# automl/CARL

Measured on AMD Instinct MI355X. Metric: env-steps/sec (whole node) at 65k parallel contexts, 1/2/4/8 MI355X, higher is better.
Workload: dtype f32

## Files before the change

carl_amd/_lib.py:

```python
from __future__ import annotations

import ctypes as C
import os

import torch

from carl_amd import build as _build

CARL_ABI_VERSION = 9
CARL_MAX_CTX_OBS = 32

CARTPOLE, PENDULUM, ACROBOT, MOUNTAINCAR, MOUNTAINCAR_CONT = range(5)
CARL_N_FAMILIES = 5
ERR_INVALID_ARGUMENT, ERR_UNSUPPORTED = -1, -2
SEL_STATIC, SEL_ROUND_ROBIN, SEL_RANDOM, SEL_HOST = range(4)
FLAG_AUTORESET = 1
FLAG_CARTPOLE_RECOMPUTE = 2
FLAG_ACROBOT_FP32 = 4
FLAG_AUTORESET_FIRST_STATE = 8
FLAG_ROLLOUT_DIRECT = 16
FLAG_BRAX_GENERIC = 32
FLAG_BRAX_FP32 = 64
ROLLOUT_STAGED, ROLLOUT_DIRECT_SHAPE, ROLLOUT_DIRECT_FLAG = range(3)
ACTION_I32, ACTION_I64, ACTION_F32, ACTION_U8, ACTION_F16, ACTION_BF16 = range(6)

_vp = C.c_void_p


class FamilyInfo(C.Structure):
    _fields_ = [
        ("state_dim", C.c_int32), ("obs_dim", C.c_int32), ("n_features", C.c_int32),
        ("action_dim", C.c_int32), ("action_is_discrete", C.c_int32), ("n_actions", C.c_int32),
        ("max_episode_steps", C.c_int32), ("reserved", C.c_int32),
        ("action_low", C.c_float), ("action_high", C.c_float),
    ]


class Batch(C.Structure):
    _fields_ = [
        ("family", C.c_int32), ("n_lanes", C.c_int32), ("n_contexts", C.c_int32),
        ("ctx_stride", C.c_int32), ("max_episode_steps", C.c_int32), ("selector", C.c_int32),
        ("selector_stride", C.c_int32), ("flags", C.c_int32),
        ("lane_offset", C.c_int64), ("seed", C.c_uint64),
        ("state", _vp), ("elapsed", _vp), ("ctx_idx", _vp), ("episode", _vp), ("n_calls", _vp),
        ("ep_return", _vp),
        ("ctx_table", _vp), ("ctx_obs", _vp),
        ("n_ctx_obs", C.c_int32), ("ctx_obs_feat", C.c_int32 * CARL_MAX_CTX_OBS),
        ("fin_capacity", C.c_int32),
        ("last_return", _vp), ("last_length", _vp), ("episodes_done", _vp),
        ("fin_count", _vp), ("fin_lane", _vp), ("fin_return", _vp), ("fin_length", _vp),
        ("goal_pos", _vp), ("success", _vp), ("first_state", _vp),
    ]


class StepIO(C.Structure):
# ... 169 lines not shown
```

carl_amd/csrc/carl_amd.hip:

```cpp
#include <hip/hip_runtime.h>

#include <cstdarg>
#include <cstdio>
#include <cstdlib>
#include <cstring>
#include <map>
#include <mutex>
#include <utility>

#include "../../include/carl_amd.h"
#include "classic_control.hip.h"
#include "context_kernels.hip.h"
#include "engine_kernels.hip.h"
#include "host_common.hpp"

namespace carl_host {

thread_local char g_err[512] = "";

int fail(int code, const char* fmt, ...) {
  va_list ap;
  va_start(ap, fmt);
  vsnprintf(g_err, sizeof g_err, fmt, ap);
  va_end(ap);
// ... 64 lines not shown
  if (io == nullptr) return fail(CARL_ERR_INVALID_ARGUMENT, "%s: io is NULL", who);
  if (!io->action || !io->obs || !io->reward || !io->terminated || !io->truncated)
    return fail(CARL_ERR_INVALID_ARGUMENT, "%s: a required io pointer is NULL", who);
  const bool discrete = kInfo[b->family].action_is_discrete != 0;
  if (discrete && io->action_dtype != CARL_ACTION_I32 && io->action_dtype != CARL_ACTION_I64 &&
      io->action_dtype != CARL_ACTION_U8)
    return fail(CARL_ERR_INVALID_ARGUMENT, "%s: discrete family needs int32/int64 (carl_rollout: or uint8) actions", who);
  if (io->action_dtype == CARL_ACTION_U8 && (reinterpret_cast<uintptr_t>(io->action) & 3) != 0)
    return fail(CARL_ERR_INVALID_ARGUMENT, "%s: uint8 actions must be 4-byte aligned", who);
  const bool half = io->action_dtype == CARL_ACTION_F16 || io->action_dtype == CARL_ACTION_BF16;
  if (!discrete && io->action_dtype != CARL_ACTION_F32 && !half)
    return fail(CARL_ERR_INVALID_ARGUMENT, "%s: continuous family needs float32 (carl_rollout: or float16 / bfloat16) actions", who);
  if (half && (reinterpret_cast<uintptr_t>(io->action) & 7) != 0)
    return fail(CARL_ERR_INVALID_ARGUMENT, "%s: float16 / bfloat16 actions must be 8-byte aligned", who);
  if (io->row_pitch != 0 && io->row_pitch < b->n_lanes)
    return fail(CARL_ERR_INVALID_ARGUMENT, "%s: io.row_pitch %d < n_lanes %d (0 = dense rows)", who, io->row_pitch, b->n_lanes);
  return 0;
}

template <class Fam>
bool use_lds_ctx(const carl_batch_t* b) {
  const size_t bytes = (size_t)Fam::F * b->n_contexts * sizeof(float);
  return bytes <= 32 * 1024 && (int64_t)b->n_contexts * 8 <= (int64_t)b->n_lanes;
}

int row_pitch_of(const carl_batch_t* b, const carl_step_io_t* io) { return io->row_pitch > 0 ? io->row_pitch : b->n_lanes; }

struct RolloutPlan {
  int variant = CARL_ROLLOUT_STAGED;
  bool lean = false;
  bool unsupported = false;
  int ak = 0;
  bool plain = false, ldsctx = false, moves = false, fin = false, ar = false, deep = false;
  size_t lds_bytes = 0;
};

template <class Fam>
RolloutPlan plan_rollout(const carl_batch_t* b, const carl_step_io_t* io) {
  static_assert(carl::predraw_of<Fam>::value, "the staged kernels below are instantiated for predrawing families");
  RolloutPlan p;
  const int dt = io->action_dtype;
  p.ak = dt == CARL_ACTION_I64 ? 1 : dt == CARL_ACTION_U8 ? carl::kActU8 : dt == CARL_ACTION_F16 ? carl::kActF16
         : dt == CARL_ACTION_BF16 ? carl::kActBF16 : 0;
  const int pitch = row_pitch_of(b, io), n16 = (b->n_lanes + 15) / 16 * 16;
  const uintptr_t bits = reinterpret_cast<uintptr_t>(io->obs) | reinterpret_cast<uintptr_t>(io->reward) |
                         reinterpret_cast<uintptr_t>(io->terminated) | reinterpret_cast<uintptr_t>(io->truncated) |
                         reinterpret_cast<uintptr_t>(io->final_obs);
  const uintptr_t amask = p.ak == carl::kActU8 ? 3u : p.ak > carl::kActU8 ? 7u : 15u;
  const bool aligned = (bits & 15) == 0 && (reinterpret_cast<uintptr_t>(io->action) & amask) == 0;
  if (b->flags & CARL_FLAG_ROLLOUT_DIRECT)
    p.variant = CARL_ROLLOUT_DIRECT_FLAG;
  else if (!(aligned && pitch % 16 == 0 && (b->n_lanes % 16 == 0 || pitch == n16)))
    p.variant = CARL_ROLLOUT_DIRECT_SHAPE;
  const bool keeps_context = b->selector == CARL_SEL_STATIC || b->selector == CARL_SEL_HOST;
  p.lean = p.variant == CARL_ROLLOUT_STAGED && keeps_context && b->fin_count == nullptr && io->final_obs == nullptr;
  p.unsupported = p.ak >= carl::kActU8 && !p.lean;
  if (p.variant != CARL_ROLLOUT_STAGED) return p;

  p.lds_bytes = carl::rollout_staged_lds_bytes<Fam>();
  const size_t table_bytes = (size_t)Fam::F * b->n_contexts * sizeof(float);
  constexpr size_t static_lds = carl::has_tables<Fam>::value ? sizeof(double) * 2 * CARL_SINCOS_TAB_N : 0;
  const bool table_fits = use_lds_ctx<Fam>(b) && p.lds_bytes + table_bytes + static_lds <= 160 * 1024;
  if (p.lean) {
    p.plain = true;
    p.ar = carl::dense_done_of<Fam>::value && (b->flags & CARL_FLAG_AUTORESET);
    p.deep = p.ak == 0 && b->n_lanes < carl::deep_below_lanes_of<Fam>::value;
  } else if (carl::dense_done_of<Fam>::value && b->fin_count == nullptr) {
    p.plain = true;
    p.moves = !keeps_context;
    p.fin = io->final_obs != nullptr;
    p.ldsctx = p.moves && table_fits;
  } else {
    p.ldsctx = !keeps_context && table_fits;
  }
  if (p.ldsctx) p.lds_bytes += table_bytes;
  return p;
}

using staged_kern_t = void (*)(carl_batch_t, carl_step_io_t, int);

template <class Fam>
staged_kern_t staged_kernel(const RolloutPlan& p) {
#define CARL_STAGED(AK, PLAIN, LDSCTX, MOVES, FIN, AR, DEEP)                                                         \
  if (p.ak == AK && p.plain == PLAIN && p.ldsctx == LDSCTX && p.moves == MOVES && p.fin == FIN && p.ar == AR &&    \
      p.deep == DEEP)                                                                                              \
    return carl::rollout_staged_kernel<Fam, AK, bool(PLAIN), bool(LDSCTX), bool(MOVES), bool(FIN), bool(AR), bool(DEEP)>;
#define CARL_STAGED_01(...) CARL_STAGED(0, __VA_ARGS__) CARL_STAGED(1, __VA_ARGS__)
  constexpr bool dense = carl::dense_done_of<Fam>::value, deep = carl::deep_below_lanes_of<Fam>::value > 0;
  CARL_STAGED_01(    0,     0,    0,  0, 0,   0)
  CARL_STAGED_01(    0,     1,    0,  0, 0,   0)
  CARL_STAGED_01(    1,     0,    0,  0, 0,   0)
  if constexpr (std::is_same_v<typename Fam::Action, int>) {
    CARL_STAGED(carl::kActU8, 1, 0, 0, 0, 0, 0)
  } else {
    CARL_STAGED(carl::kActF16, 1, 0, 0, 0, 0, 0)
    CARL_STAGED(carl::kActBF16, 1, 0, 0, 0, 0, 0)
  }
  if constexpr (deep) CARL_STAGED(0, 1, 0, 0, 0, 0, 1)
  if constexpr (dense) {
    CARL_STAGED_01(  1,     0,    0,  0, 1,   0)
    CARL_STAGED(carl::kActU8, 1, 0, 0, 0, 1, 0)
    if constexpr (deep) CARL_STAGED(0, 1, 0, 0, 0, 1, 1)
    CARL_STAGED_01(  1,     0,    0,  1, 0,   0)
    CARL_STAGED_01(  1,     0,    1,  0, 0,   0)
    CARL_STAGED_01(  1,     0,    1,  1, 0,   0)
    CARL_STAGED_01(  1,     1,    1,  0, 0,   0)
    CARL_STAGED_01(  1,     1,    1,  1, 0,   0)
  }
#undef CARL_STAGED_01
#undef CARL_STAGED
  return nullptr;
}

int pick_block(int n, bool lds) { return (lds || n > 256 * 1024) ? 256 : 64; }

template <class Fam>
int launch_reset(const carl_batch_t* b, const uint8_t* mask, const int32_t* idx, const int32_t* count, float* obs,
                 hipStream_t s) {
  if (b->n_lanes == 0) return 0;
  const bool lds = use_lds_ctx<Fam>(b);
  const int block = 256;
  int grid = (b->n_lanes + block - 1) / block;
  if (grid > 4096) grid = 4096;
  if (lds) {
    const size_t sh = (size_t)Fam::F * b->n_contexts * sizeof(float);
    hipLaunchKernelGGL((carl::reset_kernel<Fam, true>), dim3(grid), dim3(block), sh, s, *b, mask, idx, count, obs);
  } else {
    hipLaunchKernelGGL((carl::reset_kernel<Fam, false>), dim3(grid), dim3(block), 0, s, *b, mask, idx, count, obs);
  }
  return check_launch("carl_reset");
}

template <class Fam>
int launch_step(const carl_batch_t* b, const carl_step_io_t* io, int n_steps, hipStream_t s) {
  if (b->n_lanes == 0 || n_steps == 0) return 0;
  const bool rollout = n_steps >= 0;
  const RolloutPlan plan = plan_rollout<Fam>(b, io);
  if (plan.unsupported || (!rollout && plan.ak >= carl::kActU8))
    return fail(CARL_ERR_UNSUPPORTED,
                "uint8 / float16 / bfloat16 actions: carl_rollout in its lean staged configuration only (row pitch %% 16 == 0, "
                "static / host selector, no finished-episode log, no final_obs); pass int32 / int64 / float32 actions");
  carl_step_io_t io_resolved = *io;
  io_resolved.row_pitch = row_pitch_of(b, io);
  if (rollout && plan.variant == CARL_ROLLOUT_STAGED) {
    const staged_kern_t kern = staged_kernel<Fam>(plan);
    if (kern == nullptr) return fail(CARL_ERR_UNSUPPORTED, "carl_rollout: no staged kernel for this configuration");
    if (int e = carl_host::ensure_dynamic_lds(reinterpret_cast<const void*>(kern), plan.lds_bytes, "carl_rollout")) return e;
    const int grid = (b->n_lanes + carl::kRolloutLanes - 1) / carl::kRolloutLanes;
    hipLaunchKernelGGL(kern, dim3(grid), dim3(carl::kStagedThreads), plan.lds_bytes, s, *b, io_resolved, n_steps);
    return check_launch("carl_rollout");
  }
  const bool lds = use_lds_ctx<Fam>(b), a64 = io->action_dtype == CARL_ACTION_I64;
  const int block = rollout ? carl::kRolloutThreads : pick_block(b->n_lanes, lds);
  const int lanes_per_block = rollout ? carl::kRolloutLanes : block;
  const dim3 g((b->n_lanes + lanes_per_block - 1) / lanes_per_block), t(block);
  const size_t sh = (lds ? (size_t)Fam::F * b->n_contexts * sizeof(float) : 0) +
                    (rollout ? carl::rollout_action_lds_bytes() : 0);
#define CARL_LAUNCH(KERNEL, ...)                                                                    \
  do {                                                                                              \
    if (lds && a64) hipLaunchKernelGGL((carl::KERNEL<Fam, true, true>), g, t, sh, s, __VA_ARGS__);   \
    else if (lds) hipLaunchKernelGGL((carl::KERNEL<Fam, true, false>), g, t, sh, s, __VA_ARGS__);    \
    else if (a64) hipLaunchKernelGGL((carl::KERNEL<Fam, false, true>), g, t, sh, s, __VA_ARGS__);    \
    else hipLaunchKernelGGL((carl::KERNEL<Fam, false, false>), g, t, sh, s, __VA_ARGS__);            \
  } while (0)
  if (!rollout) {
    CARL_LAUNCH(step_kernel, *b, *io);
    return check_launch("carl_step");
  }
  CARL_LAUNCH(rollout_kernel, *b, io_resolved, n_steps);
#undef CARL_LAUNCH
  return check_launch("carl_rollout");
}

template <class FamB>
int launch_pair(const carl_batch_t* a, const carl_step_io_t* ioa, const carl_batch_t* b, const carl_step_io_t* iob,
                int n_steps, hipStream_t s) {
  using FamA = carl::Acrobot;
  const RolloutPlan pa = plan_rollout<FamA>(a, ioa), pb = plan_rollout<FamB>(b, iob);
  if (a->n_lanes == 0 || b->n_lanes == 0 || !pa.lean || !pb.lean || pa.ak != 0 || pb.ak != 0)
    return fail(CARL_ERR_UNSUPPORTED, "carl_rollout_pair: both parts must be lean staged rollouts (row pitch %% 16 == 0, static / host "
                "selector, no finished-episode log, no terminal observations, int32 / float32 actions)");
  using kern_t = void (*)(carl_batch_t, carl_step_io_t, carl_batch_t, carl_step_io_t, int, int);
  kern_t kern = static_cast<kern_t>(carl::rollout_staged_pair_kernel<FamA, FamB, false, false>);
  if constexpr (carl::dense_done_of<FamB>::value) {
    if (pb.ar) kern = static_cast<kern_t>(carl::rollout_staged_pair_kernel<FamA, FamB, false, true>);
  }
  const size_t sh = carl::rollout_pair_lds_bytes<FamA, FamB>();
  if (int e = carl_host::ensure_dynamic_lds(reinterpret_cast<const void*>(kern), sh, "carl_rollout_pair")) return e;
  const int grid_a = (a->n_lanes + carl::kRolloutLanes - 1) / carl::kRolloutLanes;
  const int grid_b = (b->n_lanes + carl::kRolloutLanes - 1) / carl::kRolloutLanes;
  carl_step_io_t ra = *ioa, rb = *iob;
  ra.row_pitch = row_pitch_of(a, ioa);
  rb.row_pitch = row_pitch_of(b, iob);
  hipLaunchKernelGGL(kern, dim3(grid_a + grid_b), dim3(carl::kStagedThreads), sh, s, *a, ra, *b, rb, n_steps, grid_a);
  return check_launch("carl_rollout_pair");
}

#define CARL_DISPATCH(family, CALL)                                   \
  switch (family) {                                                   \
    case CARL_CARTPOLE: return CALL(carl::CartPole);                  \
    case CARL_PENDULUM: return CALL(carl::Pendulum);                  \
    case CARL_ACROBOT:                                                \
      return (batch->flags & CARL_FLAG_ACROBOT_FP32) ? CALL(carl::AcrobotFast) : CALL(carl::Acrobot); \
    case CARL_MOUNTAINCAR: return CALL(carl::MountainCar);            \
    case CARL_MOUNTAINCAR_CONT: return CALL(carl::MountainCarCont);   \
    default: return fail(CARL_ERR_INVALID_ARGUMENT, "unknown family %d", family); \
  }

int validate_specs(const carl_feature_spec_t* sd, const carl_feature_spec_t* sh, int n_features, int n_contexts,
                   int ctx_stride, const void* table, const char* who) {
  if (sd == nullptr || sh == nullptr || table == nullptr)
// ... 85 lines not shown
    return fail(CARL_ERR_UNSUPPORTED, "carl_rollout_pair: a pair launch is Acrobot (float64) + one other family");
  if (!a_acro) {
    const carl_batch_t* tb = batch_a; batch_a = batch_b; batch_b = tb;
    const carl_step_io_t* ti = io_a; io_a = io_b; io_b = ti;
  }
  if (batch_b->family == CARL_ACROBOT)
    return fail(CARL_ERR_UNSUPPORTED, "carl_rollout_pair: the second family cannot be Acrobot");
  hipStream_t s = (hipStream_t)stream;
  switch (batch_b->family) {
    case CARL_CARTPOLE: return launch_pair<carl::CartPole>(batch_a, io_a, batch_b, io_b, n_steps, s);
    case CARL_PENDULUM: return launch_pair<carl::Pendulum>(batch_a, io_a, batch_b, io_b, n_steps, s);
    case CARL_MOUNTAINCAR: return launch_pair<carl::MountainCar>(batch_a, io_a, batch_b, io_b, n_steps, s);
    case CARL_MOUNTAINCAR_CONT: return launch_pair<carl::MountainCarCont>(batch_a, io_a, batch_b, io_b, n_steps, s);
    default: return fail(CARL_ERR_UNSUPPORTED, "carl_rollout_pair: family %d", batch_b->family);
  }
}

int carl_rollout_variant(const carl_batch_t* batch) { return carl_rollout_variant_io(batch, nullptr); }

int carl_rollout_variant_io(const carl_batch_t* batch, const carl_step_io_t* io) {
  if (batch == nullptr) {
    fail(CARL_ERR_INVALID_ARGUMENT, "carl_rollout_variant: batch is NULL");
    return CARL_ERR_INVALID_ARGUMENT;
  }
  if (batch->family < 0 || batch->family >= CARL_N_FAMILIES) {
    fail(CARL_ERR_INVALID_ARGUMENT, "carl_rollout_variant: family %d is not a classic-control family", batch->family);
    return CARL_ERR_INVALID_ARGUMENT;
  }
  if (io != nullptr && io->row_pitch != 0 && io->row_pitch < batch->n_lanes) {
    fail(CARL_ERR_INVALID_ARGUMENT, "carl_rollout_variant_io: io.row_pitch %d < n_lanes %d", io->row_pitch, batch->n_lanes);
    return CARL_ERR_INVALID_ARGUMENT;
  }
  const carl_step_io_t dense{};
#define CALL(F) plan_rollout<F>(batch, io != nullptr ? io : &dense).variant
  CARL_DISPATCH(batch->family, CALL)
#undef CALL
}

int32_t carl_rollout_pitch(int32_t n_lanes) { return n_lanes <= 0 ? 0 : (n_lanes + 15) / 16 * 16; }

int32_t carl_done_compact_scratch_elems(int32_t n) {
  return n <= 0 ? 1 : (n + carl::kCompactBlock - 1) / carl::kCompactBlock;
}

int carl_done_compact(const uint8_t* terminated, const uint8_t* truncated, int32_t n, int32_t* idx_out,
                      int32_t* count_out, int32_t* scratch, void* stream) {
  if (n < 0) return fail(CARL_ERR_INVALID_ARGUMENT, "carl_done_compact: n %d < 0", n);
  if (!count_out) return fail(CARL_ERR_INVALID_ARGUMENT, "carl_done_compact: count_out is NULL");
  if (n > 0 && (!terminated || !truncated || !idx_out || !scratch))
    return fail(CARL_ERR_INVALID_ARGUMENT, "carl_done_compact: NULL pointer");
  hipStream_t s = (hipStream_t)stream;
  if (n == 0) {
    const hipError_t e = hipMemsetAsync(count_out, 0, sizeof(int32_t), s);
    return e == hipSuccess ? 0 : fail((int)e, "carl_done_compact: %s", hipGetErrorString(e));
  }
  const int nb = carl_done_compact_scratch_elems(n);
  hipLaunchKernelGGL(carl::done_count_kernel, dim3(nb), dim3(carl::kCompactBlock), 0, s, terminated, truncated, n,
                     scratch);
  hipLaunchKernelGGL(carl::done_write_kernel, dim3(nb), dim3(carl::kCompactBlock), 0, s, terminated, truncated, n,
                     scratch, idx_out, count_out);
  return check_launch("carl_done_compact");
}

int carl_sample_contexts(const carl_feature_spec_t* specs_dev, const carl_feature_spec_t* specs_host,
                         int32_t n_features, int32_t n_contexts, int32_t ctx_stride, int64_t context_offset,
                         uint64_t seed, float* ctx_table, void* stream) {
  if (int e = validate_specs(specs_dev, specs_host, n_features, n_contexts, ctx_stride, ctx_table,
// ... 27 lines not shown
```

carl_amd/csrc/classic_control.hip.h:

```cpp
#pragma once

#include <type_traits>

#include "carl_device.hip.h"
#include "fast_math.hip.h"

namespace carl {

constexpr float kPi = 3.14159265358979323846f;

struct NoAux {};

struct CartPole {
  static constexpr int S = 4, D = 4, F = 8;
  using Action = int;
  using Aux = NoAux;
  enum { GRAVITY, MASSCART, MASSPOLE, LENGTH, FORCE_MAG, TAU, INIT_LO, INIT_HI };
  static constexpr bool kNeedsStepNoise = false;
  static constexpr bool kPredraw = true;
  static constexpr int kDeepBelowLanes = 65536;
  static constexpr bool kDenseDone = true;

  struct Params {
    float gravity, masspole, length, force_mag, tau, inv_total_mass, polemass_length;
    float init_lo, init_hi;
  };

  template <class Ctx>
  __device__ static __forceinline__ Params load(const Ctx& ctx, int c, int flags) {
    Params p;
    p.gravity = ctx.get(GRAVITY, c);
    p.masspole = ctx.get(MASSPOLE, c);
    p.length = ctx.get(LENGTH, c);
    p.force_mag = ctx.get(FORCE_MAG, c);
    p.tau = ctx.get(TAU, c);
    float total_mass;
    if (flags & CARL_FLAG_CARTPOLE_RECOMPUTE) {
      total_mass = p.masspole + ctx.get(MASSCART, c);
      p.polemass_length = p.masspole * p.length;
    } else {
      total_mass = 0.1f + 1.0f;
      p.polemass_length = 0.1f * 0.5f;
    }
    p.inv_total_mass = 1.0f / total_mass;
    p.init_lo = ctx.get(INIT_LO, c);
    p.init_hi = ctx.get(INIT_HI, c);
    return p;
  }

  __device__ static __forceinline__ void prepare(const float (&)[S], Aux&) {}

  __device__ static __forceinline__ bool out_of_bounds(float x, float theta) {
    const float x_thr = 2.4f;
    const float th_thr = (float)(12.0 * 2.0 * 3.14159265358979323846 / 360.0);
// ... 491 lines not shown
```

carl_amd/csrc/engine_kernels.hip.h:

```cpp
#pragma once

#include <type_traits>

#include "carl_device.hip.h"


namespace carl {

template <bool LDS>
using ctx_t = std::conditional_t<LDS, LdsCtx, GlobalCtx>;

template <class Fam, class = void>
struct has_tables : std::false_type {};
template <class Fam>
struct has_tables<Fam, std::void_t<decltype(Fam::kUsesSinCosTab)>> : std::bool_constant<Fam::kUsesSinCosTab> {};

template <class Fam>
__device__ __forceinline__ void stage_family_tables() {
  if constexpr (has_tables<Fam>::value) {
    Fam::stage_tables();
    __syncthreads();
  }
}

// ... 212 lines not shown
    w = select_words(r.next_ok, w, wi);
  }
  float ns[Fam::S], no[Fam::D];
  typename Fam::Aux na;
  Fam::reset(r.p, w, ns);
  Fam::prepare(ns, na);
  Fam::observe(ns, na, no);
  const bool rs = done && (b.flags & CARL_FLAG_AUTORESET) != 0;
  r.fin_return = done ? r.ep_return : r.fin_return;
  r.fin_length = done ? r.elapsed : r.fin_length;
  r.n_new_episodes += done ? 1 : 0;
#pragma unroll
  for (int j = 0; j < Fam::S; ++j) r.s[j] = rs ? ns[j] : r.s[j];
#pragma unroll
  for (int d = 0; d < Fam::D; ++d) o[d] = rs ? no[d] : o[d];
  r.aux = select_words(rs, na, r.aux);
  r.elapsed = rs ? 0 : r.elapsed;
  r.ep_return = rs ? 0.0f : r.ep_return;
  r.episode += rs ? 1u : 0u;
  r.n_new_calls += rs ? 1 : 0;
  r.next_ok = r.next_ok && !rs;
  __builtin_amdgcn_s_waitcnt(0xC07F);
}

template <class Fam, class = void>
struct deep_action_prefetch_of : std::false_type {};
template <class Fam>
struct deep_action_prefetch_of<Fam, std::void_t<decltype(Fam::kDeepActionPrefetch)>> : std::bool_constant<Fam::kDeepActionPrefetch> {};

template <class Fam, class = void>
struct deep_below_lanes_of : std::integral_constant<int, 0> {};
template <class Fam>
struct deep_below_lanes_of<Fam, std::void_t<decltype(Fam::kDeepBelowLanes)>> : std::integral_constant<int, Fam::kDeepBelowLanes> {};

template <class Fam, class = void>
struct dense_done_of : std::false_type {};
template <class Fam>
struct dense_done_of<Fam, std::void_t<decltype(Fam::kDenseDone)>> : std::bool_constant<Fam::kDenseDone> {};

template <class Fam>
struct DenseNext {
  unsigned long long ok_mask;
  float s[Fam::S];
  typename Fam::Aux aux;
  int cidx;
  typename Fam::Params p;
};

template <class Fam, class Ctx, bool MOVES>
__device__ __forceinline__ void dense_draw(const carl_batch_t& b, const Ctx& ctx, uint64_t glane,
                                           const LaneRegs<Fam>& r, unsigned long long lanes, DenseNext<Fam>& nx) {
  int cn = r.cidx;
  typename Fam::Params pn = r.p;
  if constexpr (MOVES) {
    cn = select_context(b, r.cidx, glane, r.episode);
    if (ballot(cn != r.cidx) != 0ull) {
      typename Fam::Params q = Fam::load(ctx, cn, b.flags);
      settle(q);
      pn = select_words(cn != r.cidx, q, r.p);
    }
  }
  const u32x4 w = lane_words(b.seed, glane, r.episode, kSubInit);
  float fresh[Fam::S];
  typename Fam::Aux fa;
  Fam::reset(pn, w, fresh);
  Fam::prepare(fresh, fa);
// ... 420 lines not shown
    const vf4 v = *reinterpret_cast<const vf4*>(src);
    __builtin_nontemporal_store(v, reinterpret_cast<vf4*>(dst));
  };
  for (int u = which; u < steps; u += kStorers) {
    char* rec = buf + (size_t)u * SK::kStepBytes;
    const size_t row = (size_t)(t0 + u) * n + lane_base;
    char* g_obs = reinterpret_cast<char*>(io.obs + row * Fam::D);
    char* fl = rec + SK::kFlagOff + 16 * l;
    const int fl_lane = 16 * (l & 15);
    uint8_t* fl_dst = (l < 16) ? io.terminated + row + fl_lane : io.truncated + row + fl_lane;
    if (valid == kRolloutLanes) {
#pragma unroll
      for (int off = 0; off < SK::kObsBytes; off += 1024) put(g_obs + off + 16 * l, rec + off + 16 * l);
      put(reinterpret_cast<char*>(io.reward + row) + 16 * l, rec + SK::kObsBytes + 16 * l);
      if (l < 32) put(reinterpret_cast<char*>(fl_dst), fl);
    } else {
#pragma unroll
      for (int off = 0; off < SK::kObsBytes; off += 1024)
        if (off + 16 * l < valid * Fam::D * 4) put(g_obs + off + 16 * l, rec + off + 16 * l);
      if (16 * l < valid * 4) put(reinterpret_cast<char*>(io.reward + row) + 16 * l, rec + SK::kObsBytes + 16 * l);
      if (l < 32 && fl_lane < valid) put(reinterpret_cast<char*>(fl_dst), fl);
    }
    if (l < 32) *reinterpret_cast<vf4*>(fl) = vf4{0.0f, 0.0f, 0.0f, 0.0f};
  }
}

template <class Fam, int CHUNK>
__device__ __forceinline__ void zero_flag_rows(char* out_buf, int l, int which) {
  using SK = LdsSink<Fam>;
  typedef float vf4 __attribute__((ext_vector_type(4)));
  if (l < 32)
    for (int u = which; u < 2 * CHUNK; u += kStorers)
      *reinterpret_cast<vf4*>(out_buf + (size_t)u * SK::kStepBytes + SK::kFlagOff + 16 * l) = vf4{0.0f, 0.0f, 0.0f, 0.0f};
}

template <class Fam, int A64, bool PLAIN, bool LDSCTX, bool MOVES, bool FINAL, bool AR, int CHUNK, bool DEEPALL = false>
__device__ __forceinline__ void rollout_staged_body(const carl_batch_t& b, const carl_step_io_t& io, const int n_steps,
                                                    const int wg, float* lds_dyn) {
  constexpr int kStageChunk = CHUNK;
  stage_family_tables<Fam>();
  using AStore = action_store_t<Fam, A64>;
  using Action = typename Fam::Action;
  using SK = LdsSink<Fam>;
  constexpr bool kDeep = !std::is_same_v<AStore, long long> &&
                         (DEEPALL || (deep_action_prefetch_of<Fam>::value && !std::is_same_v<AStore, Action>));
  using Pipe = ActionPipe<AStore, Action, kStageChunk, kDeep>;
  using LdsAct = typename Pipe::LdsElem;
  LdsAct* act_buf = reinterpret_cast<LdsAct*>(lds_dyn);
  char* out_buf = reinterpret_cast<char*>(lds_dyn) + (size_t)2 * kStageChunk * kRolloutLanes * sizeof(float);
  float* ctx_lds = reinterpret_cast<float*>(out_buf + (size_t)2 * kStageChunk * SK::kStepBytes);
  const ctx_t<LDSCTX> ctx = make_ctx<LDSCTX, Fam::F>(b, ctx_lds);
  const int wave = __builtin_amdgcn_readfirstlane((int)(threadIdx.x / kWave));
  const int storer = wave - (kRolloutLanes / kWave + 1);
  const bool compute = wave < kRolloutLanes / kWave;
  const bool loader = wave == kRolloutLanes / kWave;
  const int hl = threadIdx.x % kWave;
  const int lane_base = wg * kRolloutLanes;
  const int lane = lane_base + (compute ? (int)threadIdx.x : 0);
  const bool active = compute && lane < b.n_lanes;
  const uint64_t glane = (uint64_t)(b.lane_offset + lane);
  const size_t n = (size_t)io.row_pitch;
  const int n_cols = (b.n_lanes + 15) & ~15;
  const int max_steps = b.max_episode_steps;
  const AStore* act = static_cast<const AStore*>(io.action);
  constexpr int kBufActs = kStageChunk * kRolloutLanes;
  LaneRegs<Fam> r{};
// ... 102 lines not shown
      }
      }
    } else if constexpr (ROLE == 1) {
      pipe.commit(act_buf + (buf ^ 1) * kBufActs, act, n, n_cols, lane_base, hl, n_steps);
      pipe.issue(act, n, n_cols, lane_base, hl, t0 + 2 * kStageChunk, n_steps);
    } else if (t0 > 0) {
      drain_records<Fam>(out_buf + (size_t)(buf ^ 1) * kStageChunk * SK::kStepBytes, io, n, n_cols, lane_base, hl, storer,
                         t0 - kStageChunk, kStageChunk);
    }
    __syncthreads();
  }
  return buf;
  };
  const int buf = compute ? run_role(std::integral_constant<int, 0>{})
                          : loader ? run_role(std::integral_constant<int, 1>{}) : run_role(std::integral_constant<int, 2>{});
  if (compute) {
    if (active) store_lane<Fam>(b, ctx, lane, r);
  } else if (!loader) {
    const int last_t0 = ((n_steps - 1) / kStageChunk) * kStageChunk;
    drain_records<Fam>(out_buf + (size_t)(buf ^ 1) * kStageChunk * SK::kStepBytes, io, n, n_cols, lane_base, hl, storer,
                       last_t0, n_steps - last_t0);
  }
}

template <class Fam, int A64, bool PLAIN = false, bool LDSCTX = false, bool MOVES = false, bool FINAL = false,
          bool AR = false, bool DEEPALL = false>
__global__ void __launch_bounds__(kStagedThreads) rollout_staged_kernel(const carl_batch_t b, const carl_step_io_t io,
                                                                        const int n_steps) {
  extern __shared__ float lds_dyn[];
  rollout_staged_body<Fam, A64, PLAIN, LDSCTX, MOVES, FINAL, AR, kStageChunk, DEEPALL>(b, io, n_steps, (int)blockIdx.x,
                                                                                        lds_dyn);
}

constexpr int kPairChunk = 4;

template <class FamA, class FamB>
__host__ __device__ constexpr size_t rollout_pair_lds_bytes() {
  constexpr size_t a = rollout_staged_lds_bytes<FamA, kPairChunk>(), b = rollout_staged_lds_bytes<FamB, kPairChunk>();
  return a > b ? a : b;
}

template <class FamA, class FamB, bool ARA, bool ARB>
__global__ void __launch_bounds__(kStagedThreads) __attribute__((amdgpu_waves_per_eu(4)))
rollout_staged_pair_kernel(const carl_batch_t ba, const carl_step_io_t ioa, const carl_batch_t bb, const carl_step_io_t iob,
                           const int n_steps, const int grid_a) {
  extern __shared__ float lds_dyn[];
  if ((int)blockIdx.x < grid_a)
    rollout_staged_body<FamA, false, true, false, false, false, ARA && dense_done_of<FamA>::value, kPairChunk>(
        ba, ioa, n_steps, (int)blockIdx.x, lds_dyn);
  else
    rollout_staged_body<FamB, false, true, false, false, false, ARB && dense_done_of<FamB>::value, kPairChunk>(
        bb, iob, n_steps, (int)blockIdx.x - grid_a, lds_dyn);
}

constexpr int kCompactBlock = 1024;

__global__ void __launch_bounds__(kCompactBlock) done_count_kernel(const uint8_t* __restrict__ term,
                                                                    const uint8_t* __restrict__ trunc, int n,
                                                                    int32_t* __restrict__ block_counts) {
  __shared__ int wave_counts[kCompactBlock / kWave];
  const int i = blockIdx.x * kCompactBlock + threadIdx.x;
  const bool done = (i < n) && ((term[i] | trunc[i]) != 0);
  const unsigned long long m = ballot(done);
  if (lane_id() == 0) wave_counts[threadIdx.x / kWave] = __popcll(m);
  __syncthreads();
  if (threadIdx.x == 0) {
// ... 46 lines not shown
```

include/carl_amd.h:

```cpp
#ifndef CARL_AMD_H_
#define CARL_AMD_H_

#include <stdint.h>

#ifdef __cplusplus
extern "C" {
#endif

#define CARL_ABI_VERSION 9
#define CARL_MAX_CTX_OBS 32

#define CARL_ERR_INVALID_ARGUMENT (-1)
#define CARL_ERR_UNSUPPORTED (-2)

typedef enum carl_family {
  CARL_CARTPOLE = 0,
  CARL_PENDULUM = 1,
  CARL_ACROBOT = 2,
  CARL_MOUNTAINCAR = 3,
  CARL_MOUNTAINCAR_CONT = 4,
  CARL_N_FAMILIES = 5
} carl_family_t;

typedef enum carl_selector {
  CARL_SEL_STATIC = 0,
  CARL_SEL_ROUND_ROBIN = 1,
  CARL_SEL_RANDOM = 2,
  CARL_SEL_HOST = 3
} carl_selector_t;

enum {
  CARL_FLAG_AUTORESET = 1,
  CARL_FLAG_CARTPOLE_RECOMPUTE = 2,
  CARL_FLAG_ACROBOT_FP32 = 4,
  CARL_FLAG_ROLLOUT_DIRECT = 16,
  CARL_FLAG_AUTORESET_FIRST_STATE = 8
  ,
  CARL_FLAG_BRAX_GENERIC = 32
  ,
  CARL_FLAG_BRAX_FP32 = 64
};

enum { CARL_ACTION_I32 = 0, CARL_ACTION_I64 = 1, CARL_ACTION_F32 = 2, CARL_ACTION_U8 = 3,
       CARL_ACTION_F16 = 4, CARL_ACTION_BF16 = 5 };

typedef struct carl_family_info {
  int32_t state_dim;
  int32_t obs_dim;
  int32_t n_features;
  int32_t action_dim;
  int32_t action_is_discrete;
  int32_t n_actions;
  int32_t max_episode_steps;
  int32_t reserved;
  float action_low, action_high;
} carl_family_info_t;

typedef struct carl_batch {
  int32_t family;
  int32_t n_lanes;
  int32_t n_contexts;
  int32_t ctx_stride;
  int32_t max_episode_steps;
  int32_t selector;
  int32_t selector_stride;
  int32_t flags;
  int64_t lane_offset;
  uint64_t seed;
  float* state;
  int32_t* elapsed;
  int32_t* ctx_idx;
  uint32_t* episode;
  int32_t* n_calls;
// ... 190 lines not shown
```

Before: 200.4 billion.

## Add bulk action-prefetch rollout kernel packing CartPole decisions into LDS bitmasks

Adds a bulk rollout kernel for families whose action is one bit (CartPole). It reads a whole phase of actions per lane, packs them into 32-bit decision words held in LDS, and then runs the dense step chunks from those bits while storer waves drain the records. This is meant to replace per-chunk streamed action loads with batched wide reads, taking action traffic off the critical path. It uses more LDS, which may lower occupancy, and it adds two flags to force or disable the path.

```diff
diff --git a/carl_amd/_lib.py b/carl_amd/_lib.py
--- a/carl_amd/_lib.py
+++ b/carl_amd/_lib.py
@@ -21,6 +21,8 @@
 FLAG_ROLLOUT_DIRECT = 16
 FLAG_BRAX_GENERIC = 32
 FLAG_BRAX_FP32 = 64
+FLAG_ROLLOUT_STREAMED_ACTIONS = 128
+FLAG_ROLLOUT_BULK_ACTIONS = 256
 ROLLOUT_STAGED, ROLLOUT_DIRECT_SHAPE, ROLLOUT_DIRECT_FLAG = range(3)
 ACTION_I32, ACTION_I64, ACTION_F32, ACTION_U8, ACTION_F16, ACTION_BF16 = range(6)
 
diff --git a/carl_amd/csrc/carl_amd.hip b/carl_amd/csrc/carl_amd.hip
--- a/carl_amd/csrc/carl_amd.hip
+++ b/carl_amd/csrc/carl_amd.hip
@@ -120,11 +120,12 @@
   bool unsupported = false;
   int ak = 0;
   bool plain = false, ldsctx = false, moves = false, fin = false, ar = false, deep = false;
+  bool bulk = false;
   size_t lds_bytes = 0;
 };
 
 template <class Fam>
-RolloutPlan plan_rollout(const carl_batch_t* b, const carl_step_io_t* io) {
+RolloutPlan plan_rollout(const carl_batch_t* b, const carl_step_io_t* io, int n_steps) {
   static_assert(carl::predraw_of<Fam>::value, "the staged kernels below are instantiated for predrawing families");
   RolloutPlan p;
   const int dt = io->action_dtype;
@@ -161,6 +162,11 @@
   } else {
     p.ldsctx = !keeps_context && table_fits;
   }
+  if constexpr (carl::decision_bits_of<Fam>::value == 1) {
+    const bool full_chip = b->n_lanes >= carl::deep_below_lanes_of<Fam>::value || (b->flags & CARL_FLAG_ROLLOUT_BULK_ACTIONS);
+    p.bulk = p.plain && carl::dense_done_of<Fam>::value && full_chip && !(b->flags & CARL_FLAG_ROLLOUT_STREAMED_ACTIONS);
+    if (p.bulk) p.lds_bytes = carl::rollout_bulk_lds_bytes<Fam>(carl::bulk_phase_steps<Fam>(n_steps, p.ldsctx ? table_bytes : 0));
+  }
   if (p.ldsctx) p.lds_bytes += table_bytes;
   return p;
 }
@@ -169,6 +175,26 @@
 
 template <class Fam>
 staged_kern_t staged_kernel(const RolloutPlan& p) {
+  if (p.bulk) {
+    if constexpr (carl::decision_bits_of<Fam>::value == 1) {
+#define CARL_BULK(AK, LDSCTX, MOVES, FIN, AR)                                                                \
+  if (p.ak == AK && p.ldsctx == LDSCTX && p.moves == MOVES && p.fin == FIN && p.ar == AR)                \
+    return carl::rollout_bulk_kernel<Fam, AK, bool(LDSCTX), bool(MOVES), bool(FIN), bool(AR)>;
+#define CARL_BULK_01(...) CARL_BULK(0, __VA_ARGS__) CARL_BULK(1, __VA_ARGS__)
+      CARL_BULK_01(  0,    0,  0, 0)
+      CARL_BULK_01(  0,    0,  0, 1)
+      CARL_BULK(carl::kActU8, 0, 0, 0, 0)
+      CARL_BULK(carl::kActU8, 0, 0, 0, 1)
+      CARL_BULK_01(  0,    0,  1, 0)
+      CARL_BULK_01(  0,    1,  0, 0)
+      CARL_BULK_01(  0,    1,  1, 0)
+      CARL_BULK_01(  1,    1,  0, 0)
+      CARL_BULK_01(  1,    1,  1, 0)
+#undef CARL_BULK_01
+#undef CARL_BULK
+    }
+    return nullptr;
+  }
 #define CARL_STAGED(AK, PLAIN, LDSCTX, MOVES, FIN, AR, DEEP)                                                         \
   if (p.ak == AK && p.plain == PLAIN && p.ldsctx == LDSCTX && p.moves == MOVES && p.fin == FIN && p.ar == AR &&    \
       p.deep == DEEP)                                                                                              \
@@ -223,7 +249,7 @@
 int launch_step(const carl_batch_t* b, const carl_step_io_t* io, int n_steps, hipStream_t s) {
   if (b->n_lanes == 0 || n_steps == 0) return 0;
   const bool rollout = n_steps >= 0;
-  const RolloutPlan plan = plan_rollout<Fam>(b, io);
+  const RolloutPlan plan = plan_rollout<Fam>(b, io, n_steps);
   if (plan.unsupported || (!rollout && plan.ak >= carl::kActU8))
     return fail(CARL_ERR_UNSUPPORTED,
                 "uint8 / float16 / bfloat16 actions: carl_rollout in its lean staged configuration only (row pitch %% 16 == 0, "
@@ -264,7 +290,7 @@
 int launch_pair(const carl_batch_t* a, const carl_step_io_t* ioa, const carl_batch_t* b, const carl_step_io_t* iob,
                 int n_steps, hipStream_t s) {
   using FamA = carl::Acrobot;
-  const RolloutPlan pa = plan_rollout<FamA>(a, ioa), pb = plan_rollout<FamB>(b, iob);
+  const RolloutPlan pa = plan_rollout<FamA>(a, ioa, n_steps), pb = plan_rollout<FamB>(b, iob, n_steps);
   if (a->n_lanes == 0 || b->n_lanes == 0 || !pa.lean || !pb.lean || pa.ak != 0 || pb.ak != 0)
     return fail(CARL_ERR_UNSUPPORTED, "carl_rollout_pair: both parts must be lean staged rollouts (row pitch %% 16 == 0, static / host "
                 "selector, no finished-episode log, no terminal observations, int32 / float32 actions)");
@@ -416,7 +442,7 @@
     return CARL_ERR_INVALID_ARGUMENT;
   }
   const carl_step_io_t dense{};
-#define CALL(F) plan_rollout<F>(batch, io != nullptr ? io : &dense).variant
+#define CALL(F) plan_rollout<F>(batch, io != nullptr ? io : &dense, 0).variant
   CARL_DISPATCH(batch->family, CALL)
 #undef CALL
 }
diff --git a/carl_amd/csrc/classic_control.hip.h b/carl_amd/csrc/classic_control.hip.h
--- a/carl_amd/csrc/classic_control.hip.h
+++ b/carl_amd/csrc/classic_control.hip.h
@@ -20,6 +20,7 @@
   static constexpr bool kPredraw = true;
   static constexpr int kDeepBelowLanes = 65536;
   static constexpr bool kDenseDone = true;
+  static constexpr int kDecisionBits = 1;
 
   struct Params {
     float gravity, masspole, length, force_mag, tau, inv_total_mass, polemass_length;
diff --git a/carl_amd/csrc/engine_kernels.hip.h b/carl_amd/csrc/engine_kernels.hip.h
--- a/carl_amd/csrc/engine_kernels.hip.h
+++ b/carl_amd/csrc/engine_kernels.hip.h
@@ -268,6 +268,11 @@
 struct deep_below_lanes_of : std::integral_constant<int, 0> {};
 template <class Fam>
 struct deep_below_lanes_of<Fam, std::void_t<decltype(Fam::kDeepBelowLanes)>> : std::integral_constant<int, Fam::kDeepBelowLanes> {};
+
+template <class Fam, class = void>
+struct decision_bits_of : std::integral_constant<int, 0> {};
+template <class Fam>
+struct decision_bits_of<Fam, std::void_t<decltype(Fam::kDecisionBits)>> : std::integral_constant<int, Fam::kDecisionBits> {};
 
 template <class Fam, class = void>
 struct dense_done_of : std::false_type {};
@@ -754,6 +759,41 @@
   if (l < 32)
     for (int u = which; u < 2 * CHUNK; u += kStorers)
       *reinterpret_cast<vf4*>(out_buf + (size_t)u * SK::kStepBytes + SK::kFlagOff + 16 * l) = vf4{0.0f, 0.0f, 0.0f, 0.0f};
+}
+
+template <class Fam, class Ctx, bool MOVES, bool FINAL, bool AR, int CHUNK, class ActOf>
+__device__ __forceinline__ void dense_chunk(const carl_batch_t& b, const Ctx& ctx, char* rec, float* final_base, size_t n,
+                                            int t0, int steps, int max_steps_eff, bool autoreset, uint64_t glane,
+                                            LaneRegs<Fam>& r, DenseNext<Fam>& nx, ActOf act_of) {
+  using SK = LdsSink<Fam>;
+  using Action = typename Fam::Action;
+  if (nx.ok_mask != ~0ull) {
+    dense_draw<Fam, Ctx, MOVES>(b, ctx, glane, r, ~nx.ok_mask, nx);
+    nx.ok_mask = ~0ull;
+  }
+  Action acts[CHUNK];
+#pragma unroll
+  for (int u = 0; u < CHUNK; ++u) acts[u] = act_of(u);
+  if (steps == CHUNK) {
+#pragma unroll
+    for (int u = 0; u < CHUNK; ++u) {
+      const SK sink{rec + (size_t)u * SK::kStepBytes, FINAL ? final_base : nullptr, n * Fam::D, t0 + u, (int)threadIdx.x};
+      if (u == 0)
+        step_dense<Fam, Ctx, MOVES, FINAL, AR, true, SK>(b, ctx, sink, max_steps_eff, autoreset, glane, acts[u], r, nx);
+      else
+        step_dense<Fam, Ctx, MOVES, FINAL, AR, false, SK>(b, ctx, sink, max_steps_eff, autoreset, glane, acts[u], r, nx);
+    }
+  } else {
+#pragma unroll 1
+    for (int u = 0; u < steps; ++u) {
+      const SK sink{rec + (size_t)u * SK::kStepBytes, FINAL ? final_base : nullptr, n * Fam::D, t0 + u, (int)threadIdx.x};
+      Action a = acts[0];
+#pragma unroll
+      for (int k = 1; k < CHUNK; ++k) a = (u == k) ? acts[k] : a;
+      step_dense<Fam, Ctx, MOVES, FINAL, AR, true, SK>(b, ctx, sink, max_steps_eff, autoreset, glane, a, r, nx);
+    }
+  }
+  if constexpr (AR) r.n_new_calls = r.n_new_episodes;
 }
 
 template <class Fam, int A64, bool PLAIN, bool LDSCTX, bool MOVES, bool FINAL, bool AR, int CHUNK, bool DEEPALL = false>
@@ -922,6 +962,146 @@
                                                                                         lds_dyn);
 }
 
+constexpr int kDecisionRows = 8;
+
+template <class Fam>
+__host__ __device__ constexpr int bulk_phase_steps(int n_steps, size_t table_bytes) {
+  constexpr size_t kLds = 160 * 1024, records = (size_t)2 * kStageChunk * LdsSink<Fam>::kStepBytes;
+  static_assert(!has_tables<Fam>::value, "bulk_phase_steps: add the static tables to the LDS budget");
+  const int fit = (int)((kLds - records - table_bytes) / (kRolloutLanes * sizeof(unsigned))) * 32;
+  const int need = (n_steps + 31) / 32 * 32;
+  return fit < need ? fit : need;
+}
+
+template <class Fam>
+__host__ __device__ constexpr size_t rollout_bulk_lds_bytes(int phase_steps) {
+  return (size_t)2 * kStageChunk * LdsSink<Fam>::kStepBytes + (size_t)phase_steps / 32 * kRolloutLanes * sizeof(unsigned);
+}
+
+template <class Pipe, class AStore>
+__device__ __forceinline__ void read_decisions(unsigned* bits, const AStore* __restrict__ act, size_t n, int cols,
+                                               int lane_base, int wave, int l, int p0, int steps, int n_steps) {
+  static_assert(32 % kDecisionRows == 0, "a block of 32 steps is read in whole batches");
+  typedef unsigned int vu4 __attribute__((ext_vector_type(4)));
+  const int lane4 = min(lane_base + 4 * l, cols - 4);
+  const int last = n_steps - 1;
+  const int nblk = (steps + 31) / 32;
+  for (int k = wave; k < nblk; k += kStagedThreads / kWave) {
+    const int tb = p0 + 32 * k;
+    unsigned w0 = 0, w1 = 0, w2 = 0, w3 = 0;
+#pragma unroll
+    for (int s0 = 0; s0 < 32; s0 += kDecisionRows) {
+      typename Pipe::R rows[kDecisionRows];
+#pragma unroll
+      for (int u = 0; u < kDecisionRows; ++u) rows[u] = Pipe::load_row(act + (size_t)min(tb + s0 + u, last) * n + lane4);
+#pragma unroll
+      for (int u = 0; u < kDecisionRows; ++u) {
+        const auto e = Pipe::narrow(rows[u]);
+        const unsigned m = 1u << (s0 + u);
+        if constexpr (Pipe::kU8) {
+          w0 |= Pipe::widen((unsigned char)(e & 0xffu)) == 1 ? m : 0u;
+          w1 |= Pipe::widen((unsigned char)((e >> 8) & 0xffu)) == 1 ? m : 0u;
+          w2 |= Pipe::widen((unsigned char)((e >> 16) & 0xffu)) == 1 ? m : 0u;
+          w3 |= Pipe::widen((unsigned char)(e >> 24)) == 1 ? m : 0u;
+        } else {
+          w0 |= Pipe::widen(e.x) == 1 ? m : 0u;
+          w1 |= Pipe::widen(e.y) == 1 ? m : 0u;
+          w2 |= Pipe::widen(e.z) == 1 ? m : 0u;
+          w3 |= Pipe::widen(e.w) == 1 ? m : 0u;
+        }
+      }
+    }
+    *reinterpret_cast<vu4*>(bits + k * kRolloutLanes + 4 * l) = vu4{w0, w1, w2, w3};
+  }
+}
+
+template <class Fam, int A64, bool LDSCTX, bool MOVES, bool FINAL, bool AR>
+__device__ __forceinline__ void rollout_bulk_body(const carl_batch_t& b, const carl_step_io_t& io, const int n_steps,
+                                                  const int wg, float* lds_dyn) {
+  static_assert(decision_bits_of<Fam>::value == 1 && dense_done_of<Fam>::value && std::is_same_v<typename Fam::Action, int>,
+                "rollout_bulk_body: a discrete family whose step reads one bit of its action, with the dense done path");
+  stage_family_tables<Fam>();
+  using AStore = action_store_t<Fam, A64>;
+  using Action = typename Fam::Action;
+  using SK = LdsSink<Fam>;
+  using Pipe = ActionPipe<AStore, Action, kStageChunk>;
+  const int P = bulk_phase_steps<Fam>(n_steps, LDSCTX ? (size_t)Fam::F * b.n_contexts * sizeof(float) : 0);
+  char* out_buf = reinterpret_cast<char*>(lds_dyn);
+  unsigned* bits = reinterpret_cast<unsigned*>(out_buf + (size_t)2 * kStageChunk * SK::kStepBytes);
+  float* ctx_lds = reinterpret_cast<float*>(bits + (size_t)P / 32 * kRolloutLanes);
+  const ctx_t<LDSCTX> ctx = make_ctx<LDSCTX, Fam::F>(b, ctx_lds);
+  const int wave = __builtin_amdgcn_readfirstlane((int)(threadIdx.x / kWave));
+  const int storer = wave - (kRolloutLanes / kWave + 1);
+  const bool compute = wave < kRolloutLanes / kWave;
+  const int hl = threadIdx.x % kWave;
+  const int lane_base = wg * kRolloutLanes;
+  const int lane = lane_base + (compute ? (int)threadIdx.x : 0);
+  const bool active = compute && lane < b.n_lanes;
+  const uint64_t glane = (uint64_t)(b.lane_offset + lane);
+  const size_t n = (size_t)io.row_pitch;
+  const int n_cols = (b.n_lanes + 15) & ~15;
+  const AStore* act = static_cast<const AStore*>(io.action);
+  LaneRegs<Fam> r{};
+  float* const final_base = (io.final_obs != nullptr && active) ? io.final_obs + (size_t)lane * Fam::D : nullptr;
+  if (storer >= 0) {
+    zero_flag_rows<Fam, kStageChunk>(out_buf, hl, storer);
+  } else if (compute) {
+    const int src = min(lane, b.n_lanes - 1);
+    load_lane<Fam>(b, ctx, src, r);
+    if (!r.episode_valid) {
+      r.episode = b.episode[src];
+      r.episode_valid = true;
+      settle(r.episode);
+    }
+    r.valid = active;
+  }
+  auto run_role = [&](auto role_tag) -> int {
+    constexpr int ROLE = decltype(role_tag)::value;
+    int buf = 0;
+    [[maybe_unused]] DenseNext<Fam> nx{};
+    [[maybe_unused]] const bool autoreset = (b.flags & CARL_FLAG_AUTORESET) != 0;
+    [[maybe_unused]] const int max_steps_eff = b.max_episode_steps > 0 ? b.max_episode_steps : 0x7fffffff;
+    [[maybe_unused]] unsigned word = 0;
+    for (int p0 = 0; p0 < n_steps; p0 += P) {
+      const int pend = min(p0 + P, n_steps);
+      read_decisions<Pipe>(bits, act, n, n_cols, lane_base, wave, hl, p0, pend - p0, n_steps);
+      __syncthreads();
+      for (int t0 = p0; t0 < pend; t0 += kStageChunk, buf ^= 1) {
+        if constexpr (ROLE == 0) {
+          const int s = t0 - p0;
+          if ((s & 31) == 0) word = bits[(s >> 5) * kRolloutLanes + threadIdx.x];
+          const unsigned w = word >> (s & 31);
+          dense_chunk<Fam, ctx_t<LDSCTX>, MOVES, FINAL, AR, kStageChunk>(
+              b, ctx, out_buf + (size_t)buf * kStageChunk * SK::kStepBytes, final_base, n, t0, min(kStageChunk, pend - t0),
+              max_steps_eff, autoreset, glane, r, nx, [&](int u) { return (Action)((w >> u) & 1u); });
+        } else if constexpr (ROLE == 2) {
+          if (t0 > 0)
+            drain_records<Fam>(out_buf + (size_t)(buf ^ 1) * kStageChunk * SK::kStepBytes, io, n, n_cols, lane_base, hl,
+                               storer, t0 - kStageChunk, kStageChunk);
+        }
+        __syncthreads();
+      }
+    }
+    return buf;
+  };
+  const int buf = compute ? run_role(std::integral_constant<int, 0>{})
+                  : storer < 0 ? run_role(std::integral_constant<int, 1>{}) : run_role(std::integral_constant<int, 2>{});
+  if (compute) {
+    if (active) store_lane<Fam>(b, ctx, lane, r);
+  } else if (storer >= 0) {
+    const int last_t0 = ((n_steps - 1) / kStageChunk) * kStageChunk;
+    drain_records<Fam>(out_buf + (size_t)(buf ^ 1) * kStageChunk * SK::kStepBytes, io, n, n_cols, lane_base, hl, storer,
+                       last_t0, n_steps - last_t0);
+  }
+}
+
+template <class Fam, int A64, bool LDSCTX = false, bool MOVES = false, bool FINAL = false, bool AR = false>
+__global__ void __launch_bounds__(kStagedThreads) rollout_bulk_kernel(const carl_batch_t b, const carl_step_io_t io,
+                                                                      const int n_steps) {
+  extern __shared__ float lds_dyn[];
+  rollout_bulk_body<Fam, A64, LDSCTX, MOVES, FINAL, AR>(b, io, n_steps, (int)blockIdx.x, lds_dyn);
+}
+
 constexpr int kPairChunk = 4;
 
 template <class FamA, class FamB>
diff --git a/include/carl_amd.h b/include/carl_amd.h
--- a/include/carl_amd.h
+++ b/include/carl_amd.h
@@ -39,6 +39,10 @@
   CARL_FLAG_BRAX_GENERIC = 32
   ,
   CARL_FLAG_BRAX_FP32 = 64
+  ,
+  CARL_FLAG_ROLLOUT_STREAMED_ACTIONS = 128
+  ,
+  CARL_FLAG_ROLLOUT_BULK_ACTIONS = 256
 };
 
 enum { CARL_ACTION_I32 = 0, CARL_ACTION_I64 = 1, CARL_ACTION_F32 = 2, CARL_ACTION_U8 = 3,
```

Measured after the change: 225.7 billion, median of 6. 12.6% higher.
